# InSilicoModellingGroup/rdcFEs

Measured on AMD Instinct MI355X. Metric: elements_assembled_per_sec, higher is better.
Workload: dtype f64; 1 GPU; PIHNA TET4 K(119): 10110954 tets, 1728000 nodes, 5 unknowns, params run/PIHNA/input.dat (shipped), order=lex, state of SURVEY App. C (background (0,0,0,7170,0) of the shipped field file, tumour values inside a sphere r = 0.25; see state_sensitivity); scatter=rowgather, kernel_variant=auto, parallelism=single GPU, rank0_local_elements=10110954, rank0_nnz=639395950

## Files before the change

rdcfes_amd/csrc/rdc_capi.hip:

```cpp
#include <algorithm>
#include <cmath>
#include <cstdarg>
#include <cstdio>
#include <cstring>
#include <new>
#include <type_traits>
#include <utility>

#include "rdc_internal.h"
#include "rdc_const_rows.h"
#include "rdc_parts.h"
#include "rdc_tet4_ev.h"
#include "rdc_tet4_cl.h"
#include "rdc_solid.h"
#include "rdc_solve.h"

using namespace rdc;

namespace {

struct DevBuf { void* p = nullptr; size_t bytes = 0; bool owned = true; };

struct Buffers {
  struct { DevBuf conn, xyz, bptr, eslot, elem_order, first_mask, first_rhs, pair_elem, pair_local, node_pair_ptr, wg_node_ptr; } mesh;
// ... 58 lines not shown
  bool solid_part1_pending = false;
  int32_t n_materials = 0;
  int64_t n_sides = 0;
  int64_t field_count[RDC_FIELD_COUNT] = {};
};

thread_local char g_create_error[512] = "";

}

struct rdc_ctx {
  int device = 0;
  hipStream_t stream = nullptr;
  char err[512] = "";
  int strategy = RDC_SCATTER_AUTO;
  int variant = RDC_VARIANT_AUTO;
  int tet4_cl_mode = 0;
  int tet4_cl_active = 0;
  size_t tet4_cl_lds = 0;
  Options opt;
  MeshState ms;
  Buffers buf;
  ConstRows const_rows;
  hipEvent_t pack_event = nullptr;
  hipStream_t copy_stream = nullptr;
  hipEvent_t copy_fence = nullptr;
  static constexpr int N_TICKETS = 16;
  hipEvent_t ticket[N_TICKETS] = {};
  int next_ticket = 0;
  hipEvent_t solid_part1_event = nullptr;
  SolveScal* solve_rec = nullptr;
  int mg_omega_permille = MG_OMEGA_PERMILLE;
  int mg_smoother = 0;
  int mg_gs_fuse = 1;
  int ilu_factor_bits = 64;
  int solve_method = 0;
  int gmres_restart = GMRES_DEFAULT_RESTART;
  int gmres_refine = 0;
  GmresRec* gmres_rec = nullptr;
  bool timing = false;
  std::vector<hipEvent_t> ev;
  size_t ev_used = 0;
  size_t max_lds = 64 * 1024;
  int n_cu = 256;
};

// ... 409 lines not shown
  }
  a.val = (double*)c->buf.out.val.p;
  a.rhs = (double*)c->buf.out.rhs.p;
  a.stream = c->stream;
  a.colour_ptr = c->ms.prep.colour_ptr.data();
  a.n_colours = c->ms.prep.n_colours;
  a.n_wg = c->ms.prep.rowgather_ok ? (int)c->ms.prep.wg_node_ptr.size() - 1 : 0;
  a.lds_bytes = c->ms.prep.rg_lds_bytes;
  a.ev_start = nullptr;
  hipEvent_t ev_stop = nullptr;
  if (c->timing) {
    if ((rc = next_event_pair(c, &a.ev_start, &ev_stop))) return rc;
  }
  ConstRowsKey rows_key;
  bool capturing = false;
  if constexpr (std::is_same<M, Pihna>::value) {
    if (const_rows_path) {
      rows_key = const_rows_key(k);
      hipStreamCaptureStatus cs = hipStreamCaptureStatusNone;
      if (hipStreamIsCapturing(c->stream, &cs) != hipSuccess) { (void)hipGetLastError(); capturing = true; }
      else capturing = cs != hipStreamCaptureStatusNone;
      a.ev_rows = c->const_rows.rows(c->const_rows.mode, rows_key, plan.two_part == TwoPart::WHOLE ? 0 : part, c->opt.interior_nodes, capturing);
    }
  }
  hipError_t e = launch_specialised<M>(a, k);
  if (const_rows_path) c->const_rows.launched(a.ev_rows, rows_key, plan.two_part == TwoPart::WHOLE ? 0 : part, capturing, e == hipSuccess);
  if (e != hipSuccess) return fail(c, RDC_ERR_HIP, "kernel launch failed: %s", hipGetErrorString(e));
  if (c->timing) RDC_HIP(c, hipEventRecord(ev_stop, c->stream));
  return RDC_OK;
}

template <class F>
int with_part(rdc_ctx* c, int part, void* stream, F&& call) {
  if (!c) return RDC_ERR_INVALID;
  if (part < 0 || part > 2) return fail(c, RDC_ERR_INVALID, "part must be 0, 1 or 2");
  const int part0 = c->opt.part;
  const hipStream_t s0 = c->stream;
  c->opt.part = part;
  c->stream = (hipStream_t)stream;
  const int rc = call();
  c->opt.part = part0;
  c->stream = s0;
  return rc;
}
}

// ... 101 lines not shown
  if (!std::strcmp(key, "ilu_factor_bits")) {
    if (value != 64 && value != 32) return fail(c, RDC_ERR_INVALID, "ilu_factor_bits is 64 or 32, not %d", value);
    c->ilu_factor_bits = value;
    return RDC_OK;
  }
  if (!std::strcmp(key, "solve_method")) {
    if (value != 0 && value != 1) return fail(c, RDC_ERR_INVALID, "solve_method is 0 (BiCGStab) or 1 (GMRES), not %d", value);
    c->solve_method = value;
    return RDC_OK;
  }
  if (!std::strcmp(key, "gmres_restart")) {
    if (value < 1 || value > GMRES_MAX_RESTART) return fail(c, RDC_ERR_INVALID, "gmres_restart is 1 .. %d, not %d", GMRES_MAX_RESTART, value);
    c->gmres_restart = value;
    return RDC_OK;
  }
  if (!std::strcmp(key, "gmres_refine")) {
    if (value != 0 && value != 1) return fail(c, RDC_ERR_INVALID, "gmres_refine is 0 or 1, not %d", value);
    c->gmres_refine = value;
    return RDC_OK;
  }
  if (!std::strcmp(key, "const_rows")) {
    if (!const_rows_mode_ok(value)) return fail(c, RDC_ERR_INVALID, "%s", CONST_ROWS_REFUSED);
    c->const_rows.mode = value;
    return RDC_OK;
  }
  return options_set(c->opt, key, value, c->err, sizeof(c->err));
}

int rdc_get_scatter(const rdc_ctx* c, int* s) {
  if (!c || !s) return RDC_ERR_INVALID;
  int r = c->strategy;
  if (r == RDC_SCATTER_AUTO && c->ms.have_mesh) r = c->ms.prep.rowgather_ok ? RDC_SCATTER_ROWGATHER : RDC_SCATTER_COLOURED;
  *s = r;
  return RDC_OK;
}

int rdc_mesh_upload(rdc_ctx* c, int elem_type, int64_t n_elem, int64_t n_node, int64_t n_owned,
                    const uint32_t* conn, const double* xyz, int nvar) {
  if (!c) return RDC_ERR_INVALID;
  if (!conn || !xyz) return fail(c, RDC_ERR_INVALID, "null mesh arrays");
  int rc = set_device(c);
  if (rc) return rc;
  c->ms.have_mesh = false;
  c->const_rows.mesh_upload();
  const size_t budget = c->max_lds >= 64 * 1024 ? 50 * 1024 : c->max_lds / 2;
  std::string err = prep_build(elem_type, n_elem, n_node, n_owned, conn, nvar, budget, c->opt.block, c->ms.prep, c->opt.schedule != 0);
// ... 1415 lines not shown
```

rdcfes_amd/csrc/rdc_integrands.h:

```cpp
#ifndef RDC_INTEGRANDS_H
#define RDC_INTEGRANDS_H

#include <math.h>
#include "../../include/rdc_assembly.h"

#if defined(__HIPCC__)
#define RDC_HD __host__ __device__ __forceinline__
#else
#define RDC_HD inline
#endif

namespace rdc {

template <int NV, int NG>
struct Coef {
  double A[NV][NV];
  double B[NV][NV][NG];
  double D[NV][NV];
  double R[NV];
  double RG[NV][NG];
  RDC_HD void zero() {
    for (int a = 0; a < NV; a++) {
      R[a] = 0.0;
      for (int k = 0; k < NG; k++) RG[a][k] = 0.0;
// ... 36 lines not shown
  else if (EXP_MODE == 2) { pm1 = x; p = x * x; }
  else if (EXP_MODE == 3) { pm1 = x * x; p = pm1 * x; }
  else if (EXP_MODE == 4) { pm1 = x * x * x; p = pm1 * x; }
  else if (EXP_MODE == 25) { pm1 = x * sqrt(x); p = pm1 * x; }
  else {
    if (e == 3.0) { pm1 = x * x; p = pm1 * x; }
    else if (e == 2.0) { pm1 = x; p = x * x; }
    else if (e == 2.5) { pm1 = x * sqrt(x); p = pm1 * x; }
    else if (e == 4.0) { pm1 = x * x * x; p = pm1 * x; }
    else if (e == 1.0) { pm1 = 1.0; p = x; }
    else { p = rdc_pow_pos(x, e); pm1 = p * rcp(x); }
  }
}

struct PihnaK {
  double DT2, Lambda, Kappa, Ka, ek;
  double iKappa, mekK;
  double nec_c, nec_h, nec_v;
  double dif_c, tax_c, dif_h, tax_h, prod_c, c2h, h2c, h2n;
  double dif_v, tax_v, prod_v;
  double sec_c, sec_h, upt, dec;
  double Tn_c, Tn_h, Tn_v, Th2n, Tprod_c, Tc2h, Th2c, Tprod_v, Tdif_v, Tsec_c, Tsec_h, Tupt, Tdec;
  double Tdif_c, Ttax_c, Tdif_h, Ttax_h, Ttax_v;
};

struct Pihna {
  static constexpr int HEX_CL_POINTS = 1;
  static constexpr bool HEX_STAGED = false;
  static constexpr bool HEX_REF_GRADS = true;
  static constexpr int AUX_LOCAL_NODE = -1;
  static constexpr int NELEM = 0;
  RDC_HD static void grad_post(const PihnaK&, double (*)[3], const double*) {}
  static constexpr int NV = 5, NG = 4, NAUX = 0;
  static constexpr int FAST_EXP_MODE = 3;
  using K = PihnaK;
  using C = Coef<NV, NG>;
  RDC_HD static constexpr int grad_src(int k) { return k + 1; }
  RDC_HD static constexpr int row_order(int x) { return x; }
  RDC_HD static constexpr bool hasA(int a, int b) {
    return !((a == 0 && b == 4) || (a == 4 && b == 0) || (a == 1 && b == 4) || (a == 2 && b == 4));
  }
  RDC_HD static constexpr bool hasB(int a, int b, int k) {
    return b < 4 && ((a == 1 && (k == 0 || k == 2)) || (a == 2 && (k == 1 || k == 2)) || (a == 3 && (k == 2 || k == 3)));
  }
  RDC_HD static constexpr bool hasD(int a, int b) {
    return (a == 1 && (b == 1 || b == 3)) || (a == 2 && (b == 2 || b == 3)) || (a == 3 && (b == 3 || b == 4));
// ... 3 lines not shown
  }

  static inline K derive(const rdc_pihna_params& p) {
    K k;
    k.DT2 = p.time_step / 2.0;
    k.Lambda = p.cells_min_capacity;
    k.Kappa = p.cells_max_capacity;
    k.Ka = p.cytokines_max_capacity;
    k.ek = p.cells_max_capacity_exponent;
    k.iKappa = 1.0 / k.Kappa;
    k.mekK = -k.ek / k.Kappa;
    k.nec_c = p.necrosis_c / k.Kappa;
    k.nec_h = p.necrosis_h / k.Kappa;
    k.nec_v = p.necrosis_v / k.Kappa;
    k.dif_c = p.diffuse_c; k.tax_c = p.taxis_c; k.dif_h = p.diffuse_h; k.tax_h = p.taxis_h;
    k.prod_c = p.produce_c; k.c2h = p.switch_c2h; k.h2c = p.switch_h2c; k.h2n = p.switch_h2n;
    k.dif_v = p.diffuse_v; k.tax_v = p.taxis_v; k.prod_v = p.produce_v;
    k.sec_c = p.secrete_a_c; k.sec_h = p.secrete_a_h; k.upt = p.uptake_a_v; k.dec = p.decay_a;
    k.Tn_c = k.DT2 * k.nec_c; k.Tn_h = k.DT2 * k.nec_h; k.Tn_v = k.DT2 * k.nec_v; k.Th2n = k.DT2 * k.h2n;
    k.Tprod_c = k.DT2 * k.prod_c; k.Tc2h = k.DT2 * k.c2h; k.Th2c = k.DT2 * k.h2c; k.Tprod_v = k.DT2 * k.prod_v;
    k.Tdif_v = k.DT2 * k.dif_v; k.Tsec_c = k.DT2 * k.sec_c; k.Tsec_h = k.DT2 * k.sec_h; k.Tupt = k.DT2 * k.upt;
    k.Tdec = k.DT2 * k.dec;
    k.Tdif_c = k.DT2 * k.dif_c; k.Ttax_c = k.DT2 * k.tax_c; k.Tdif_h = k.DT2 * k.dif_h; k.Ttax_h = k.DT2 * k.tax_h; k.Ttax_v = k.DT2 * k.tax_v;
    return k;
  }
  static inline double exponent(const K& k) { return k.ek; }

  struct Pt {
    double n, c, h, v, a;
    double Tau, dT;
    double Ve, rV;
  };

  template <int EXP_MODE>
  RDC_HD static void point(const K& k, const double* u, const double* , Pt& s) {
    s.n = u[0]; s.c = u[1]; s.h = u[2]; s.v = u[3]; s.a = u[4];
    const double Te = (s.n + s.c + s.h + s.v) * k.iKappa;
    if (Te <= 0.0) { s.Tau = 1.0; s.dT = 0.0; }
    else if (Te >= 1.0) { s.Tau = 0.0; s.dT = 0.0; }
    else {
      double p, pm1;
      pow_pair<EXP_MODE>(1.0 - Te, k.ek, p, pm1);
      s.Tau = p;
      s.dT = k.mekK * pm1;
    }
    const double chv = s.c + s.h + s.v;
// ... 700 lines not shown
```

rdcfes_amd/csrc/rdc_internal.h:

```cpp
#ifndef RDC_INTERNAL_H
#define RDC_INTERNAL_H

#include <hip/hip_runtime.h>
#include <stdint.h>
#include <atomic>
#include <string>
#include <type_traits>
#include <vector>

#include "rdc_kernels.h"
#include "rdc_models.h"
#include "rdc_options.h"
#include "rdc_prep.h"

namespace rdc {

inline void dyn_lds_once(std::atomic<uint64_t>& done, const void* fn, int bytes) {
  int dev = 0;
  (void)hipGetDevice(&dev);
  const uint64_t bit = dev >= 0 && dev < 64 ? (1ull << dev) : 0;
  if (bit && (done.load(std::memory_order_relaxed) & bit)) return;
  (void)hipFuncSetAttribute(fn, hipFuncAttributeMaxDynamicSharedMemorySize, bytes);
  if (bit) done.fetch_or(bit, std::memory_order_relaxed);
}
// ... 42 lines not shown
};

struct LaunchArgs {
  MeshDev m;
  int nen, exp_mode;
  const double* u;
  const double* aux;
  const int64_t* hx_nl_ptr = nullptr;
  const uint32_t* hx_nlist = nullptr;
  const uint16_t* hx_ploc = nullptr;
  int hx_max_nodes = 0;
  const double* elem = nullptr;
  double* packed;
  int pack_part = 0;
  hipEvent_t pack_event = nullptr;
  Options opt;
  Plan plan;
  Rg2Dev rg2;
  EvDev ev;
  ClDev cl;
  int ev_grid = 0;
  int* ev_ticket = nullptr;
  int ev_rows = 5;
  long long* stamps = nullptr;
  double* val;
  double* rhs;
  hipStream_t stream;
  hipEvent_t ev_start;
  const int64_t* colour_ptr;
  int n_colours;
  int n_wg;
  size_t lds_bytes;
};

template <class M>
hipError_t launch_rd(const LaunchArgs& a, const typename M::K& k);
template <class M>
hipError_t launch_tet4_fast(const LaunchArgs& a, const typename M::K& k);
template <class M>
hipError_t launch_tet4_cl(const LaunchArgs& a, const typename M::K& k);
hipError_t pack_nodes_pihna(const LaunchArgs& a);
hipError_t launch_tet4_ev(const LaunchArgs& a, const PihnaK& k);
template <class M>
hipError_t launch_tet4_evc(const LaunchArgs& a, const typename M::K& k);

}
// ... 2 lines not shown
```

rdcfes_amd/csrc/rdc_tet4_ev.h:

```cpp
#ifndef RDC_TET4_EV_H
#define RDC_TET4_EV_H
#include "rdc_integrands.h"

namespace rdc {
namespace ev {

constexpr int NM = 16;
constexpr int NMG = 22;
constexpr int NBP = 256;
constexpr int MAXN = 16;
enum { M_E1, M_EoV, M_EPh, M_EQh, M_En, M_Ec, M_Eh, M_Ev, M_Ea, M_Ex, M_Ey, M_ETau, M_EdTc, M_Epv, M_Eg4, M_Edd,
       M_Xc, M_Yc, M_Zc, M_Xh, M_Yh, M_Zh };
constexpr bool symmetric_moment(int m) { return m != M_Epv; }
constexpr bool symmetric_moment_gen(int m) { return m != M_Epv && m != M_Edd && m != M_Xc && m != M_Yc && m != M_Xh && m != M_Yh; }

template <int EXP_MODE, class Sink, bool MIRROR = true, bool GEN = false>
RDC_HD void pihna_visit(const PihnaK& k, const double (&X)[4][3], const double (&U)[4][5], const int r, Sink& sink, const bool bg = false) {
  double e1[3], e2[3], e3[3];
#pragma unroll
  for (int d = 0; d < 3; d++) { e1[d] = X[1][d] - X[0][d]; e2[d] = X[2][d] - X[0][d]; e3[d] = X[3][d] - X[0][d]; }
  double g[4][3];
  g[1][0] = e2[1] * e3[2] - e2[2] * e3[1]; g[1][1] = e2[2] * e3[0] - e2[0] * e3[2]; g[1][2] = e2[0] * e3[1] - e2[1] * e3[0];
  g[2][0] = e3[1] * e1[2] - e3[2] * e1[1]; g[2][1] = e3[2] * e1[0] - e3[0] * e1[2]; g[2][2] = e3[0] * e1[1] - e3[1] * e1[0];
  g[3][0] = e1[1] * e2[2] - e1[2] * e2[1]; g[3][1] = e1[2] * e2[0] - e1[0] * e2[2]; g[3][2] = e1[0] * e2[1] - e1[1] * e2[0];
  const double det = e1[0] * g[1][0] + e1[1] * g[1][1] + e1[2] * g[1][2];
  const double inv = rcp(det), inv2 = inv * inv;
  const double adet = fabs(det);
#pragma unroll
  for (int d = 0; d < 3; d++) g[0][d] = -(g[1][d] + g[2][d] + g[3][d]);
  const double Wc = adet * (-2.0 / 15.0), Wh = adet * 0.075;
  const double a0 = Wc * (1.0 / 16.0), b36 = Wh * (1.0 / 36.0), w18 = Wh * (1.0 / 18.0);
  Pihna::Pt s[5];
  {
    double S[5];
#pragma unroll
    for (int v = 0; v < 5; v++) S[v] = (U[0][v] + U[1][v]) + (U[2][v] + U[3][v]);
#pragma unroll
    for (int q = 0; q < 5; q++) {
      double uq[5];
#pragma unroll
      for (int v = 0; v < 5; v++) uq[v] = (q == 0) ? 0.25 * S[v] : (S[v] * (1.0 / 6.0) + U[q == 0 ? 0 : q - 1][v] * (1.0 / 3.0));
      Pihna::point<EXP_MODE>(k, uq, nullptr, s[q]);
    }
  }
#define RDC_EV_SYM(m, beta)                                                                              \
  {                                                                                                      \
    const double Sm_ = a0 * beta[0] + b36 * ((beta[1] + beta[2]) + (beta[3] + beta[4]));                 \
    const double t_[4] = {w18 * beta[1], w18 * beta[2], w18 * beta[3], w18 * beta[4]};                   \
    _Pragma("unroll") for (int i = 0; i < 4; i++) if (i < r) {                                           \
      const double rb_ = Sm_ + t_[i];                                                                    \
      _Pragma("unroll") for (int j = 0; j < 4; j++) if (!MIRROR || j >= i) sink.mom(m, i, j, j == i ? rb_ + 3.0 * t_[i] : rb_ + t_[j]); \
    }                                                                                                    \
  }
#define RDC_EV_PT(name, expr) double name[5]; _Pragma("unroll") for (int q = 0; q < 5; q++) name[q] = (expr);
  const double o0 = Wc * 0.25, o6 = Wh * (1.0 / 6.0), o3 = Wh * (1.0 / 3.0);
#define RDC_EV_RHS(a, G)                                                             \
    {                                                                                \
      const double base_ = o0 * G[0] + o6 * ((G[1] + G[2]) + (G[3] + G[4]));         \
      _Pragma("unroll") for (int i = 0; i < 4; i++) if (i < r) sink.rhs(a, i, base_ + o3 * G[i + 1]); \
    }
  {
    double uav[5];
    {
      double g4[5];
#pragma unroll
      for (int q = 0; q < 5; q++) {
        const double raK = rcp(s[q].a + k.Ka);
        const double Ua = s[q].a * raK, Ua_da = raK - Ua * raK;
        uav[q] = Ua * s[q].v;
        g4[q] = -k.Tprod_v * (s[q].Tau * Ua_da * s[q].v);
      }
      RDC_EV_SYM(M_Eg4, g4)
    }
    {
      RDC_EV_PT(G3, s[q].v + k.Tprod_v * (s[q].Tau * uav[q]) - k.Tn_v * (s[q].v * s[q].n))
// ... 143 lines not shown
    }
  }
  if (!bg) {
    RDC_EV_PT(G, s[q].a + k.Tsec_c * s[q].c + k.Tsec_h * s[q].h - k.Tupt * (s[q].v * s[q].a) - k.Tdec * s[q].a)
    RDC_EV_RHS(4, G)
  }
#undef RDC_EV_RHS
  {
    const double one[5] = {1.0, 1.0, 1.0, 1.0, 1.0};
    RDC_EV_SYM(M_E1, one)
  }
  if (!bg) {
    { RDC_EV_PT(b, s[q].n) RDC_EV_SYM(M_En, b) }
    { RDC_EV_PT(b, s[q].c) RDC_EV_SYM(M_Ec, b) }
    { RDC_EV_PT(b, s[q].h) RDC_EV_SYM(M_Eh, b) }
    { RDC_EV_PT(b, s[q].dT * s[q].c) RDC_EV_SYM(M_EdTc, b) }
  }
  { RDC_EV_PT(b, s[q].v) RDC_EV_SYM(M_Ev, b) }
  if (k.Tupt != 0.0) { RDC_EV_PT(b, s[q].a) RDC_EV_SYM(M_Ea, b) }
  { RDC_EV_PT(b, s[q].Tau) RDC_EV_SYM(M_ETau, b) }
#undef RDC_EV_SYM
#undef RDC_EV_PT
}

RDC_HD bool pihna_background(const double (&U)[4][5]) {
  bool b = true;
#pragma unroll
  for (int j = 0; j < 4; j++) b = b && U[j][0] == 0.0 && U[j][1] == 0.0 && U[j][2] == 0.0 && U[j][4] == 0.0 && U[j][3] > 0.0;
  return b;
}

template <int NMT>
RDC_HD void pihna_expand(const PihnaK& k, const double (&e)[NMT], double (&o)[25]) {
  const double E1 = e[M_E1], EoV = e[M_EoV], EPh = e[M_EPh], EQh = e[M_EQh], En = e[M_En], Ec = e[M_Ec], Eh = e[M_Eh], Ev = e[M_Ev];
  const double x = e[M_Ex], y = e[M_Ey], pcj = k.Tprod_c * e[M_EdTc], pv = e[M_Epv];
  o[0] = E1 - k.Tn_c * Ec - k.Tn_h * Eh - k.Tn_v * Ev;
  o[1] = -(k.Tn_c * En + k.Th2n * EPh);
  o[2] = -(k.Tn_h * En + k.Th2n * EPh + k.Th2n * EoV);
  o[3] = k.Th2n * EQh - k.Tn_v * En;
  o[4] = 0.0;
  o[5] = k.Tn_c * Ec - pcj;
  o[6] = E1 - k.Tprod_c * e[M_ETau] - pcj + k.Tc2h * EoV + x + k.Tn_c * En;
  o[7] = x - pcj - k.Th2c * (E1 - EoV);
  o[8] = -(pcj + y);
  o[9] = 0.0;
  const double x2 = x - k.Th2n * EPh;
  o[10] = k.Tn_h * Eh;
  o[11] = -(k.Tc2h * EoV + x2);
  o[12] = E1 - x2 + k.Th2c * (E1 - EoV) + k.Tn_h * En + k.Th2n * EoV;
  o[13] = y - k.Th2n * EQh;
  o[14] = 0.0;
  o[15] = pv + k.Tn_v * Ev;
// ... 20 lines not shown
```

rdcfes_amd/csrc/rdc_tet4_ev.hip:

```cpp
#include "rdc_internal.h"
#include <type_traits>
#include "rdc_tet4_ev.h"
#include "rdc_ev_phases.h"

namespace rdc {

template <int ABL_>
struct EvSink {
  static constexpr int ABL = ABL_ == 4 ? 0 : ABL_;
  double* p[4][4];
  double* pr[4];
  double sum = 0.0;
  __device__ __forceinline__ void mom(int m, int i, int j, double v) {
    if (ABL == 0) __hip_atomic_fetch_add(p[i][j] + m * ev::NBP, v, __ATOMIC_RELAXED, __HIP_MEMORY_SCOPE_WORKGROUP);
    else if (ABL == 1) p[i][j][m * ev::NBP] = v;
    else sum += v;
  }
  __device__ __forceinline__ void rhs(int a, int i, double v) {
    if (ABL == 0) __hip_atomic_fetch_add(pr[i] + a * ev::MAXN, v, __ATOMIC_RELAXED, __HIP_MEMORY_SCOPE_WORKGROUP);
    else if (ABL == 1) pr[i][a * ev::MAXN] = v;
    else sum += v;
  }
};


namespace {
template <bool GEN, int NM>
__device__ __forceinline__ void ev_read_moments(const double* lds, const int blk, const int mirror, double (&e)[NM]) {
  constexpr auto sym = [](const int m) { return GEN ? ev::symmetric_moment_gen(m) : ev::symmetric_moment(m); };
  constexpr int NS = [=]() { int n = 0; for (int m = 0; m < NM; m++) n += sym(m); return n; }();
#pragma unroll
  for (int m = 0; m < NM; m++) e[m] = lds[m * ev::NBP + blk];
  if (mirror != blk) {
    double t[NS];
#pragma unroll
    for (int m = 0, x = 0; m < NM; m++)
      if (sym(m)) t[x++] = lds[m * ev::NBP + mirror];
    evl::lds_batch();
    evl::lds_land(t);
#pragma unroll
    for (int m = 0, x = 0; m < NM; m++)
      if (sym(m)) e[m] += t[x++];
  }
}
}

template <int EXP_MODE, int MINW, int ABL = 0, bool GEN = false, int NROW = 5>
__global__ void __launch_bounds__(256, MINW)
k_tet4_ev(const HostPrepEv::Desc* __restrict__ desc, const uint32_t* __restrict__ nlist, const uint32_t* __restrict__ vloc,
          const uint32_t* __restrict__ vslot, const HostPrepEv::Node* __restrict__ ntab, const uint8_t* __restrict__ bpart,
          const uint32_t* __restrict__ wg_perm, const PihnaK k, const double* __restrict__ rec, double* __restrict__ val,
          double* __restrict__ rhs, const int nls, const int wg_begin, const int xcd_n, const int stagger,
          long long* __restrict__ stamps, const int bg_skip) {
  static_assert(NROW == 4 || NROW == 5, "all five equation rows, or all but the a row");
  constexpr int BLOCK = 256, NP = 4;
  constexpr bool TL = ABL == 4;
  long long ts[11];
#define RDC_TS(x) if (TL) ts[x] = __builtin_amdgcn_s_memtime()
  RDC_TS(0);
  constexpr int NM = GEN ? ev::NMG : ev::NM, NBP = ev::NBP, MAXN = ev::MAXN;
  extern __shared__ __attribute__((aligned(16))) double lds[];
  __shared__ __attribute__((aligned(16))) HostPrepEv::Node snode[MAXN];
  typedef __attribute__((address_space(3))) void* lds_ptr;
  typedef const __attribute__((address_space(1))) void* glb_ptr;
  if (stagger > 0 && blockIdx.x < 1024u) {
    const unsigned lds_base = __builtin_amdgcn_s_getreg((7 << 11) | 6);
    const uint32_t slot = lds_base == 0 ? 0u : (lds_base < 144u ? 1u : 2u);
    for (uint32_t i = 0; i < slot * (uint32_t)stagger; i++) __builtin_amdgcn_s_sleep(16);
  }
  int wl = (int)blockIdx.x;
  if (xcd_n > 0) {
    const int q = xcd_n >> 3, rem = xcd_n & 7, x = wl & 7;
    wl = x * q + (x < rem ? x : rem) + (wl >> 3);
  }
  int w = wl + wg_begin;
  if (wg_perm) w = (int)wg_perm[w];
  const int tid = threadIdx.x, lane = tid & 63, wv = tid >> 6;
  double* const R = lds + NM * NBP;
  double* const recs = R + 5 * MAXN;
  evl::zero_slice<NM * NBP * 8>(lds, __builtin_amdgcn_readfirstlane(wv));
  if (tid < 5 * MAXN) lds[NM * NBP + tid] = 0.0;
  const int rounds = nls >> 6;
  uint32_t nid = 0;
  if (wv < rounds) nid = nlist[(size_t)w * nls + wv * 64 + lane];
  const uint32_t pl = vloc[(size_t)w * BLOCK + tid];
  const uint2 sl = reinterpret_cast<const uint2*>(vslot)[(size_t)w * BLOCK + tid];
  const HostPrepEv::Desc d = desc[w];
  const int mirror = (int)bpart[(size_t)w * NBP + tid];
  if (tid < MAXN) snode[tid] = ntab[(size_t)w * MAXN + tid];
  if (wv < rounds) {
    const char* src = reinterpret_cast<const char*>(rec) + (size_t)nid * (NP * 16);
#pragma unroll
    for (int p = 0; p < NP; p++)
      __builtin_amdgcn_global_load_lds((glb_ptr)(src + p * 16), (lds_ptr)evl::rec_at(recs, nls, p, wv * 64), 16, 0, 0);
  }
  RDC_TS(1);
  asm volatile("s_waitcnt vmcnt(0)" ::: "memory");
  RDC_TS(2);
  __syncthreads();
  RDC_TS(3);
  if (pl != evl::IDLE) {
    double X[4][3], U[4][5];
    int li[4];
#pragma unroll
    for (int j = 0; j < 4; j++) {
      li[j] = evl::vloc_pos(pl, j);
      double rr[2 * NP];
#pragma unroll
      for (int p = 0; p < NP; p++) {
        const double2 v2 = evl::rec_piece(recs, nls, p, li[j]);
        rr[2 * p] = v2.x; rr[2 * p + 1] = v2.y;
      }
      X[j][0] = rr[0]; X[j][1] = rr[1]; X[j][2] = rr[2];
#pragma unroll
      for (int v = 0; v < 5; v++) U[j][v] = rr[3 + v];
    }
    const int r = evl::vloc_rows(li, (int)d.nown);
    EvSink<ABL> sink;
    evl::aim(sink, lds, R, li, r, sl);
    const bool bg = bg_skip && __builtin_amdgcn_ballot_w64(!ev::pihna_background(U)) == 0;
    if (ABL != 3) ev::pihna_visit<EXP_MODE, EvSink<ABL>, true, GEN>(k, X, U, r, sink, bg);
    if (ABL == 2 && sink.sum == 1.2345e300) rhs[0] = sink.sum;
  }
  if (TL) asm volatile("s_waitcnt lgkmcnt(0)" ::: "memory");
  RDC_TS(4);
  __syncthreads();
  RDC_TS(5);
  double e[NM];
  const int bn = evl::block_node(tid), bs = evl::block_slot(tid);
  const bool has = bn < (int)d.nown && bs < (int)snode[bn < (int)d.nown ? bn : 0].len;
  if (has) ev_read_moments<GEN>(lds, tid, mirror, e);
  if (tid < (int)d.nown * 5) {
    const int n = tid / 5, a = tid - n * 5;
    rhs[(size_t)snode[n].node * 5 + a] = R[a * MAXN + n];
  }
  RDC_TS(6);
  __syncthreads();
  if (has) {
    double o[25];
    ev::pihna_expand(k, e, o);
    const int len = (int)snode[bn].len;
    double* dst = lds + snode[bn].obase + evl::seg_entry(5, len, 0, bs, 0);
#pragma unroll
    for (int a = 0; a < NROW; a++)
#pragma unroll
      for (int b = 0; b < 5; b++) dst[evl::seg_entry(5, len, a, 0, b)] = o[a * 5 + b];
  }
  RDC_TS(7);
  __syncthreads();
  RDC_TS(8);
  {
    const int wvu = __builtin_amdgcn_readfirstlane(wv);
    HostPrepEv::Node nd[4];
    evl::wave_nodes(snode, wvu, nd);
// ... 24 lines not shown
}
}
namespace {
struct EvqLists {
  static constexpr int PL = 0, SL = 1024, MISC = SL + 2048, MIRROR = MISC, SNODE = MISC + 256, DESC = MISC + 512, NL = MISC + 544;
  static constexpr int bytes(int nls) { return NL + 2 * nls * 4; }
};
}
template <int EXP_MODE, bool TL, bool GEN = false, int NROW = 5>
__global__ void __launch_bounds__(256, GEN ? 2 : 3)
k_tet4_evq(const HostPrepEv::Desc* __restrict__ desc, const uint32_t* __restrict__ nlist, const uint32_t* __restrict__ vloc,
           const uint32_t* __restrict__ vslot, const HostPrepEv::Node* __restrict__ ntab, const uint8_t* __restrict__ bpart,
           const PihnaK k, const double* __restrict__ rec, double* __restrict__ val, double* __restrict__ rhs, const int nls,
           const int wg_begin, const int wg_count, long long* __restrict__ stamps, const int bg_skip, int* __restrict__ ticket,
           const uint32_t* __restrict__ wg_perm) {
  static_assert(NROW == 4 || NROW == 5, "k_tet4_ev");
  constexpr int BLOCK = 256, NP = 4;
  constexpr int NM = GEN ? ev::NMG : ev::NM, NBP = ev::NBP, MAXN = ev::MAXN;
  extern __shared__ __attribute__((aligned(16))) double lds[];
  __shared__ __attribute__((aligned(16))) HostPrepEv::Node snode[MAXN];
  __shared__ uint8_t smirror[NBP];
  __shared__ int s_nown;
  __shared__ int s_tk[2];
  double* const R = lds + NM * NBP;
  double* const recs = R + 5 * MAXN;
  char* const lists = reinterpret_cast<char*>(recs + (size_t)NP * nls * 2);
  const int rounds = nls >> 6;
  auto lds_barrier = [&]() { asm volatile("s_waitcnt lgkmcnt(0)\n\ts_barrier" ::: "memory"); };
  const int wv = __builtin_amdgcn_readfirstlane((int)(threadIdx.x >> 6));
  constexpr int NONE = 0x7fffffff;
  int c0 = (int)blockIdx.x, c1 = c0 + (int)gridDim.x, c2 = c0 + 2 * (int)gridDim.x;
  auto cluster_of = [&](const int c) -> int { return c < wg_count ? (wg_perm ? (int)wg_perm[wg_begin + c] : wg_begin + c) : -1; };
  int w0c = cluster_of(c0), w1c = cluster_of(c1), w2c = cluster_of(c2);
#define RDC_TS(x) if (TL && stamps && c0 < wg_count && lane == 0) stamps[((int64_t)c0 * 4 + wv) * 12 + x] = __builtin_amdgcn_s_memtime()
  auto fetch = [&](const int w, const uint32_t nid, const int w2, const int nb2, const int lane) {
    if (wv < rounds) {
      const char* src = reinterpret_cast<const char*>(rec) + (size_t)nid * (NP * 16);
#pragma unroll
      for (int p = 0; p < NP; p++) evl_dma16(src + p * 16, evl::rec_at(recs, nls, p, wv * 64));
    }
    if (wv == 0) evl_dma16(reinterpret_cast<const char*>(vloc + (size_t)w * BLOCK) + lane * 16, lists + EvqLists::PL);
    else if (wv < 3) evl_dma16(reinterpret_cast<const char*>(vslot + (size_t)w * BLOCK * 2) + (wv - 1) * 1024 + lane * 16, lists + EvqLists::SL + (wv - 1) * 1024);
    else {
      if (lane < 34) {
        const char* src = lane < 16 ? reinterpret_cast<const char*>(bpart + (size_t)w * NBP) + lane * 16
                        : lane < 32 ? reinterpret_cast<const char*>(ntab + (size_t)w * MAXN) + (lane - 16) * 16
                                    : reinterpret_cast<const char*>(desc + w) + (lane - 32) * 16;
        evl_dma16(src, lists + EvqLists::MISC);
      }
      if (w2 >= 0 && lane < (nls >> 2)) evl_dma16(reinterpret_cast<const char*>(nlist + (size_t)w2 * nls) + lane * 16, lists + EvqLists::NL + nb2 * nls * 4);
    }
  };
  {
    uint32_t nid0 = 0;
    if (wv < rounds) nid0 = nlist[(size_t)w0c * nls + threadIdx.x];
    asm volatile("s_waitcnt vmcnt(0)" : "+v"(nid0)::"memory");
    fetch(w0c, nid0, w1c, 1, (int)(threadIdx.x & 63));
  }
  int tk = NONE;
  bool pending = false;
#pragma unroll 1
  for (int it = 0;; it++) {
    int lane;
    asm volatile("v_mbcnt_lo_u32_b32 %0, -1, 0\n\tv_mbcnt_hi_u32_b32 %0, -1, %0" : "=v"(lane));
    RDC_TS(0);
    evl::zero_slice<NM * NBP * 8>(lds, wv);
    if (wv * 64 + lane < 5 * MAXN) lds[NM * NBP + wv * 64 + lane] = 0.0;
    asm volatile("s_waitcnt vmcnt(0)" : "+v"(tk)::"memory");
    if (pending && wv == 0 && lane == 0) s_tk[0] = tk == NONE ? NONE : 3 * (int)gridDim.x + tk;
    RDC_TS(1);
    lds_barrier();
    RDC_TS(2);
    if (pending) { c2 = __builtin_amdgcn_readfirstlane(s_tk[0]); w2c = cluster_of(c2); }
    if (c0 >= wg_count) break;
    {
      const int tid = wv * 64 + lane;
      const uint32_t pl = *reinterpret_cast<const uint32_t*>(lists + EvqLists::PL + tid * 4);
      const uint2 sl = *reinterpret_cast<const uint2*>(lists + EvqLists::SL + tid * 8);
      const int nown = (int)reinterpret_cast<const HostPrepEv::Desc*>(lists + EvqLists::DESC)->nown;
      {
        const int blk = evl::block(((wv >> 1) << 3) | (lane & 7), ((wv & 1) << 3) | (lane >> 3));
        smirror[blk] = *reinterpret_cast<const uint8_t*>(lists + EvqLists::MIRROR + blk);
        if (tid < MAXN) snode[tid] = *reinterpret_cast<const HostPrepEv::Node*>(lists + EvqLists::SNODE + tid * 16);
        if (tid == 0) s_nown = nown;
      }
      if (pl != evl::IDLE) {
        double X[4][3], U[4][5];
        int li[4];
#pragma unroll
        for (int j = 0; j < 4; j++) {
          li[j] = evl::vloc_pos(pl, j);
          double rr[2 * NP];
#pragma unroll
          for (int p = 0; p < NP; p++) {
            const double2 v2 = evl::rec_piece(recs, nls, p, li[j]);
            rr[2 * p] = v2.x; rr[2 * p + 1] = v2.y;
          }
          X[j][0] = rr[0]; X[j][1] = rr[1]; X[j][2] = rr[2];
#pragma unroll
          for (int v = 0; v < 5; v++) U[j][v] = rr[3 + v];
        }
        const int r = evl::vloc_rows(li, nown);
        EvSink<0> sink;
        evl::aim(sink, lds, R, li, r, sl);
        const bool bg = bg_skip && __builtin_amdgcn_ballot_w64(!ev::pihna_background(U)) == 0;
        ev::pihna_visit<EXP_MODE, EvSink<0>, true, GEN>(k, X, U, r, sink, bg);
      }
    }
    RDC_TS(3);
    lds_barrier();
    RDC_TS(4);
    asm volatile("v_mbcnt_lo_u32_b32 %0, -1, 0\n\tv_mbcnt_hi_u32_b32 %0, -1, %0" : "=v"(lane));
    const int bn = ((wv >> 1) << 3) | (lane & 7), bs = ((wv & 1) << 3) | (lane >> 3), blk = evl::block(bn, bs);
    int nown = s_nown, mirror = (int)smirror[blk];
    uint32_t bn_len = reinterpret_cast<const uint32_t*>(snode + bn)[1], bn_obase = snode[bn].obase;
    uint32_t base8 = snode[8].obase;
    uint32_t nid = 0;
    if (c1 < wg_count && wv < rounds) nid = *reinterpret_cast<const uint32_t*>(lists + EvqLists::NL + (((it + 1) & 1) * nls + wv * 64 + lane) * 4);
    evl::lds_batch();
    evl::lds_land(nown, mirror); evl::lds_land(bn_len, bn_obase); evl::lds_land(base8, nid);
    nown = __builtin_amdgcn_readfirstlane(nown);
    base8 = __builtin_amdgcn_readfirstlane(base8);
    bn_len &= 0xFFFFu;
    if (c1 < wg_count) fetch(w1c, nid, w2c, it & 1, lane);
    tk = NONE;
    if (c2 < wg_count && wv == 0 && lane == 0) {
      const int one = 1;
      asm volatile("global_atomic_add %0, %1, %2, off sc0" : "=v"(tk) : "v"(ticket), "v"(one) : "memory");
    }
    pending = true;
    double e[NM];
    const bool has = bn < nown && bs < (int)bn_len;
#pragma unroll
    for (int m = 0; m < NM; m++) e[m] = 0.0;
    if (has) ev_read_moments<GEN>(lds, blk, mirror, e);
    {
      const int tid = wv * 64 + lane;
      if (tid < nown * 5) {
        const int n = tid / 5, a = tid - n * 5;
        rhs[(size_t)snode[n].node * 5 + a] = R[a * MAXN + n];
      }
    }
    double o[25];
    ev::pihna_expand(k, e, o);
    lds_barrier();
#pragma unroll 1
    for (int h = 0; h < 2; h++) {
      const int n0 = h * 8;
      if (n0 >= nown) break;
      const uint32_t base = h == 0 ? 0u : (base8 & ~1u);
      if ((wv >> 1) == h && has) {
        const int len = (int)bn_len;
        double* dst = lds + (bn_obase - base) + evl::seg_entry(5, len, 0, bs, 0);
#pragma unroll
        for (int a = 0; a < NROW; a++)
#pragma unroll
          for (int b = 0; b < 5; b++) dst[evl::seg_entry(5, len, a, 0, b)] = o[a * 5 + b];
      }
      evl::v4u_t raw[2];
      evl::wave_nodes_read(snode, n0 + wv, raw);
      HostPrepEv::Node ndh[2];
      evl::wave_nodes_land(raw, ndh);
      lds_barrier();
      const int n1 = nown < n0 + 8 ? nown : n0 + 8;
      const bool on[2] = {n0 + wv < n1, n0 + wv + 4 < n1};
      if (on[0]) evl::store_segments<25, 2, 5 * NROW>(lds, val, ndh, on, lane, base);
      lds_barrier();
    }
    RDC_TS(5);
    if (TL && lane == 0 && stamps) {
      long long* op = stamps + ((int64_t)c0 * 4 + wv) * 12;
      op[11] = (long long)__builtin_amdgcn_s_getreg((31 << 11) | 4) | ((long long)__builtin_amdgcn_s_getreg((31 << 11) | 20) << 32);
    }
    c0 = c1; c1 = c2; w0c = w1c; w1c = w2c;
  }
#undef RDC_TS
}


namespace {
template <int MODE, int MINW, int ABL, bool GEN>
hipError_t launch_ev(const LaunchArgs& a, const PihnaK& k, const int wg_count, const size_t lds_bytes) {
  const EvDev& E = a.ev;
  auto kern = k_tet4_ev<MODE, MINW, ABL, GEN, 5>;
  if constexpr (ABL == 0 || ABL == 4) {
    if (a.ev_rows == 4) kern = k_tet4_ev<MODE, MINW, ABL, GEN, 4>;
  } else if (a.ev_rows != 5) return hipErrorInvalidValue;
  hipLaunchKernelGGL(kern, dim3(wg_count), dim3(256), lds_bytes, a.stream, E.desc, E.nlist, E.vloc, E.vslot, E.ntab,
                     E.bpart, E.wg_perm, k, a.packed, a.val, a.rhs, E.nls, E.wg_begin, a.opt.xcd ? wg_count : 0, a.opt.stagger, a.stamps, a.opt.ev_background);
  return hipGetLastError();
}
template <int MODE, bool TL, bool GEN>
hipError_t launch_evq(const LaunchArgs& a, const PihnaK& k, const int wg_count, const int grid, const size_t lds_bytes) {
  const EvDev& E = a.ev;
  const auto kern = a.ev_rows == 4 ? k_tet4_evq<MODE, TL, GEN, 4> : k_tet4_evq<MODE, TL, GEN, 5>;
  hipLaunchKernelGGL(kern, dim3(grid), dim3(256), lds_bytes, a.stream, E.desc, E.nlist, E.vloc, E.vslot, E.ntab, E.bpart, k,
                     a.packed, a.val, a.rhs, E.nls, E.wg_begin, wg_count, a.stamps, a.opt.ev_background, a.ev_ticket + (a.pack_part == 2 ? 16 : 0), E.wg_perm);
  return hipGetLastError();
}
}

hipError_t launch_tet4_ev(const LaunchArgs& a, const PihnaK& k) {
  const EvDev& E = a.ev;
  hipError_t e = pack_nodes_pihna(a);
  if (e != hipSuccess) return e;
  if (a.ev_start) (void)hipEventRecord(a.ev_start, a.stream);
  const int wg_count = E.wg_count < 0 ? E.n_wg - E.wg_begin : E.wg_count;
  if (wg_count <= 0) return hipSuccess;
  const size_t acc = (size_t)(a.plan.ev_general ? ev::NMG : ev::NM) * ev::NBP + 5 * ev::MAXN + (size_t)4 * E.nls * 2;
  const bool cube = a.exp_mode == 3;
  const int evq_grid = a.opt.grid > 0 ? a.opt.grid : (a.ev_grid > 0 ? (a.plan.ev_general ? a.ev_grid : a.ev_grid / 2 * 3) : 768);
  if (a.opt.ev_resident && (!a.opt.ablate || (a.opt.ablate == 4 && !a.plan.ev_general)) && a.opt.ev_occupancy == 3 && !a.opt.xcd && a.opt.stagger == 0 &&
      (a.opt.grid > 0 || a.opt.ev_resident == 2 || (int64_t)wg_count >= 56 * (int64_t)evq_grid)) {
    const int grid = evq_grid > wg_count ? wg_count : evq_grid;
    const size_t bytes = acc * sizeof(double) + EvqLists::bytes(E.nls);
    if (!a.ev_ticket) return hipErrorInvalidValue;
    if (a.plan.ev_general) return cube ? launch_evq<3, false, true>(a, k, wg_count, grid, bytes) : launch_evq<0, false, true>(a, k, wg_count, grid, bytes);
    else if (a.opt.ablate == 4) return cube ? launch_evq<3, true, false>(a, k, wg_count, grid, bytes) : launch_evq<0, true, false>(a, k, wg_count, grid, bytes);
    else return cube ? launch_evq<3, false, false>(a, k, wg_count, grid, bytes) : launch_evq<0, false, false>(a, k, wg_count, grid, bytes);
  }
// ... 14 lines not shown
```

Measured before the change: 7.509 billion elements/s.

## Add wave-uniform background fast path folding constant-state moments per block

Adds a fast path in the TET4 element-visit assembly for waves whose elements all sit in the uniform background state, meaning zero cells and the same vasculature value at every node. Such waves skip the five per-quadrature-point material evaluations and emit only the geometric moment plus the diffusion and RHS terms. Background-dependent scalars are computed once, parked in shared memory, and folded into the moments at readout. This cuts transcendental and arithmetic work for the large background region, at the cost of an extra ballot and uniformity check per wave, added code size and register pressure, and a dependence on shared-memory state whose ordering is subtle.

```diff
diff --git a/rdcfes_amd/csrc/rdc_capi.hip b/rdcfes_amd/csrc/rdc_capi.hip
--- a/rdcfes_amd/csrc/rdc_capi.hip
+++ b/rdcfes_amd/csrc/rdc_capi.hip
@@ -104,6 +104,7 @@
   MeshState ms;
   Buffers buf;
   ConstRows const_rows;
+  int ev_uniform = 1;
   hipEvent_t pack_event = nullptr;
   hipStream_t copy_stream = nullptr;
   hipEvent_t copy_fence = nullptr;
@@ -559,6 +560,7 @@
       else capturing = cs != hipStreamCaptureStatusNone;
       a.ev_rows = c->const_rows.rows(c->const_rows.mode, rows_key, plan.two_part == TwoPart::WHOLE ? 0 : part, c->opt.interior_nodes, capturing);
     }
+    if (plan.path == Path::TET4_EV) a.ev_uniform = ev::pihna_uniform_allowed(k, plan.ev_general, c->opt.ev_background, c->opt.ablate, c->ev_uniform);
   }
   hipError_t e = launch_specialised<M>(a, k);
   if (const_rows_path) c->const_rows.launched(a.ev_rows, rows_key, plan.two_part == TwoPart::WHOLE ? 0 : part, capturing, e == hipSuccess);
@@ -706,6 +708,10 @@
   if (!std::strcmp(key, "const_rows")) {
     if (!const_rows_mode_ok(value)) return fail(c, RDC_ERR_INVALID, "%s", CONST_ROWS_REFUSED);
     c->const_rows.mode = value;
+    return RDC_OK;
+  }
+  if (!std::strcmp(key, "ev_uniform")) {
+    c->ev_uniform = value ? 1 : 0;
     return RDC_OK;
   }
   return options_set(c->opt, key, value, c->err, sizeof(c->err));
diff --git a/rdcfes_amd/csrc/rdc_integrands.h b/rdcfes_amd/csrc/rdc_integrands.h
--- a/rdcfes_amd/csrc/rdc_integrands.h
+++ b/rdcfes_amd/csrc/rdc_integrands.h
@@ -82,6 +82,7 @@
   double sec_c, sec_h, upt, dec;
   double Tn_c, Tn_h, Tn_v, Th2n, Tprod_c, Tc2h, Th2c, Tprod_v, Tdif_v, Tsec_c, Tsec_h, Tupt, Tdec;
   double Tdif_c, Ttax_c, Tdif_h, Ttax_h, Ttax_v;
+  double iKa;
 };
 
 struct Pihna {
@@ -131,6 +132,7 @@
     k.Tdif_v = k.DT2 * k.dif_v; k.Tsec_c = k.DT2 * k.sec_c; k.Tsec_h = k.DT2 * k.sec_h; k.Tupt = k.DT2 * k.upt;
     k.Tdec = k.DT2 * k.dec;
     k.Tdif_c = k.DT2 * k.dif_c; k.Ttax_c = k.DT2 * k.tax_c; k.Tdif_h = k.DT2 * k.dif_h; k.Ttax_h = k.DT2 * k.tax_h; k.Ttax_v = k.DT2 * k.tax_v;
+    k.iKa = 1.0 / k.Ka;
     return k;
   }
   static inline double exponent(const K& k) { return k.ek; }
diff --git a/rdcfes_amd/csrc/rdc_internal.h b/rdcfes_amd/csrc/rdc_internal.h
--- a/rdcfes_amd/csrc/rdc_internal.h
+++ b/rdcfes_amd/csrc/rdc_internal.h
@@ -88,6 +88,7 @@
   int ev_grid = 0;
   int* ev_ticket = nullptr;
   int ev_rows = 5;
+  bool ev_uniform = false;
   long long* stamps = nullptr;
   double* val;
   double* rhs;
diff --git a/rdcfes_amd/csrc/rdc_tet4_ev.h b/rdcfes_amd/csrc/rdc_tet4_ev.h
--- a/rdcfes_amd/csrc/rdc_tet4_ev.h
+++ b/rdcfes_amd/csrc/rdc_tet4_ev.h
@@ -15,7 +15,8 @@
 constexpr bool symmetric_moment_gen(int m) { return m != M_Epv && m != M_Edd && m != M_Xc && m != M_Yc && m != M_Xh && m != M_Yh; }
 
 template <int EXP_MODE, class Sink, bool MIRROR = true, bool GEN = false>
-RDC_HD void pihna_visit(const PihnaK& k, const double (&X)[4][3], const double (&U)[4][5], const int r, Sink& sink, const bool bg = false) {
+RDC_HD void pihna_visit_u(const PihnaK& k, const double (&X)[4][3], const double (&U)[4][5], const int r, Sink& sink, const bool bg, const bool uni,
+                          const double v0) {
   double e1[3], e2[3], e3[3];
 #pragma unroll
   for (int d = 0; d < 3; d++) { e1[d] = X[1][d] - X[0][d]; e2[d] = X[2][d] - X[0][d]; e3[d] = X[3][d] - X[0][d]; }
@@ -30,19 +31,6 @@
   for (int d = 0; d < 3; d++) g[0][d] = -(g[1][d] + g[2][d] + g[3][d]);
   const double Wc = adet * (-2.0 / 15.0), Wh = adet * 0.075;
   const double a0 = Wc * (1.0 / 16.0), b36 = Wh * (1.0 / 36.0), w18 = Wh * (1.0 / 18.0);
-  Pihna::Pt s[5];
-  {
-    double S[5];
-#pragma unroll
-    for (int v = 0; v < 5; v++) S[v] = (U[0][v] + U[1][v]) + (U[2][v] + U[3][v]);
-#pragma unroll
-    for (int q = 0; q < 5; q++) {
-      double uq[5];
-#pragma unroll
-      for (int v = 0; v < 5; v++) uq[v] = (q == 0) ? 0.25 * S[v] : (S[v] * (1.0 / 6.0) + U[q == 0 ? 0 : q - 1][v] * (1.0 / 3.0));
-      Pihna::point<EXP_MODE>(k, uq, nullptr, s[q]);
-    }
-  }
 #define RDC_EV_SYM(m, beta)                                                                              \
   {                                                                                                      \
     const double Sm_ = a0 * beta[0] + b36 * ((beta[1] + beta[2]) + (beta[3] + beta[4]));                 \
@@ -51,6 +39,39 @@
       const double rb_ = Sm_ + t_[i];                                                                    \
       _Pragma("unroll") for (int j = 0; j < 4; j++) if (!MIRROR || j >= i) sink.mom(m, i, j, j == i ? rb_ + 3.0 * t_[i] : rb_ + t_[j]); \
     }                                                                                                    \
+  }
+  if (!GEN && uni) {
+    const double u0[5] = {0.0, 0.0, 0.0, v0, 0.0};
+    Pihna::Pt s0;
+    Pihna::point<EXP_MODE>(k, u0, nullptr, s0);
+    {
+      const double one[5] = {1.0, 1.0, 1.0, 1.0, 1.0};
+      RDC_EV_SYM(M_Ea, one)
+    }
+    const double sdd = k.Tdif_v * (s0.v > k.Lambda ? s0.Tau : 0.0) * (Wc + 4.0 * Wh) * inv2;
+    const double fv = s0.v * (Wc * 0.25 + Wh);
+#pragma unroll
+    for (int i = 0; i < 4; i++) if (i < r) {
+      const double gs[3] = {sdd * g[i][0], sdd * g[i][1], sdd * g[i][2]};
+#pragma unroll
+      for (int j = 0; j < 4; j++)
+        if (!MIRROR || j >= i) sink.mom(M_Edd, i, j, gs[0] * g[j][0] + gs[1] * g[j][1] + gs[2] * g[j][2]);
+      sink.rhs(3, i, fv);
+    }
+    return;
+  }
+  Pihna::Pt s[5];
+  {
+    double S[5];
+#pragma unroll
+    for (int v = 0; v < 5; v++) S[v] = (U[0][v] + U[1][v]) + (U[2][v] + U[3][v]);
+#pragma unroll
+    for (int q = 0; q < 5; q++) {
+      double uq[5];
+#pragma unroll
+      for (int v = 0; v < 5; v++) uq[v] = (q == 0) ? 0.25 * S[v] : (S[v] * (1.0 / 6.0) + U[q == 0 ? 0 : q - 1][v] * (1.0 / 3.0));
+      Pihna::point<EXP_MODE>(k, uq, nullptr, s[q]);
+    }
   }
 #define RDC_EV_PT(name, expr) double name[5]; _Pragma("unroll") for (int q = 0; q < 5; q++) name[q] = (expr);
   const double o0 = Wc * 0.25, o6 = Wh * (1.0 / 6.0), o3 = Wh * (1.0 / 3.0);
@@ -240,12 +261,51 @@
 #undef RDC_EV_SYM
 #undef RDC_EV_PT
 }
+template <int EXP_MODE, class Sink, bool MIRROR = true, bool GEN = false>
+RDC_HD void pihna_visit(const PihnaK& k, const double (&X)[4][3], const double (&U)[4][5], const int r, Sink& sink, const bool bg = false,
+                        const double* uni = nullptr) {
+  pihna_visit_u<EXP_MODE, Sink, MIRROR, GEN>(k, X, U, r, sink, bg, uni != nullptr, uni != nullptr ? *uni : 0.0);
+}
 
 RDC_HD bool pihna_background(const double (&U)[4][5]) {
   bool b = true;
 #pragma unroll
   for (int j = 0; j < 4; j++) b = b && U[j][0] == 0.0 && U[j][1] == 0.0 && U[j][2] == 0.0 && U[j][4] == 0.0 && U[j][3] > 0.0;
   return b;
+}
+
+RDC_HD bool pihna_uniform(const double (&U)[4][5], const double v0) {
+  return U[0][3] == v0 && U[1][3] == v0 && U[2][3] == v0 && U[3][3] == v0;
+}
+
+inline bool pihna_uniform_allowed(const PihnaK& k, const bool gen, const int ev_background, const int ablate, const int ev_uniform) {
+  return !gen && k.Tupt == 0.0 && k.Ka > 0.0 && k.Ka <= 1.7976931348623157e308 && ev_background != 0 && (ablate == 0 || ablate == 4) &&
+         ev_uniform != 0;
+}
+
+template <int EXP_MODE>
+RDC_HD void pihna_uniform_scalars(const PihnaK& k, const double v0, double (&u)[3]) {
+  const double u0[5] = {0.0, 0.0, 0.0, v0, 0.0};
+  Pihna::Pt s0;
+  Pihna::point<EXP_MODE>(k, u0, nullptr, s0);
+  u[0] = s0.v;
+  u[1] = s0.Tau;
+  u[2] = -k.Tprod_v * (s0.Tau * k.iKa * s0.v);
+}
+
+template <int NMT>
+RDC_HD void pihna_fold_uniform(const double (&u)[3], double (&e)[NMT]) {
+  const double Eu = e[M_Ea];
+  e[M_E1] += Eu;
+  e[M_Ev] += u[0] * Eu;
+  e[M_ETau] += u[1] * Eu;
+  e[M_Eg4] += u[2] * Eu;
+}
+template <int EXP_MODE, int NMT>
+RDC_HD void pihna_fold_uniform(const PihnaK& k, const double v0, double (&e)[NMT]) {
+  double u[3];
+  pihna_uniform_scalars<EXP_MODE>(k, v0, u);
+  pihna_fold_uniform(u, e);
 }
 
 template <int NMT>
diff --git a/rdcfes_amd/csrc/rdc_tet4_ev.hip b/rdcfes_amd/csrc/rdc_tet4_ev.hip
--- a/rdcfes_amd/csrc/rdc_tet4_ev.hip
+++ b/rdcfes_amd/csrc/rdc_tet4_ev.hip
@@ -42,6 +42,53 @@
     for (int m = 0, x = 0; m < NM; m++)
       if (sym(m)) e[m] += t[x++];
   }
+}
+
+constexpr int EV_BG = 1, EV_UNI = 2;
+
+template <int EXP_MODE>
+__device__ __forceinline__ bool ev_wave_uniform(const PihnaK& k, const double (&U)[4][5], const double v0, double* park) {
+  if (!__builtin_isfinite(v0) || __builtin_amdgcn_ballot_w64(!ev::pihna_uniform(U, v0)) != 0) return false;
+  double u[3];
+  ev::pihna_uniform_scalars<EXP_MODE>(k, v0, u);
+  const uint64_t act = __builtin_amdgcn_ballot_w64(true);
+  if (__builtin_amdgcn_mbcnt_hi((uint32_t)(act >> 32), __builtin_amdgcn_mbcnt_lo((uint32_t)act, 0u)) == 0) {
+    park[0] = u[0]; park[1] = u[1]; park[2] = u[2];
+  }
+  return true;
+}
+
+template <int EXP_MODE, int ABL, bool GEN>
+__device__ __forceinline__ void ev_visit(const PihnaK& k, const uint32_t pl, const uint2 sl, const int nown, double* lds, double* R, const double* recs,
+                                         const int nls, const int bg_skip, double* park, EvSink<ABL>& sink) {
+  double X[4][3], U[4][5];
+  int li[4];
+#pragma unroll
+  for (int j = 0; j < 4; j++) {
+    li[j] = evl::vloc_pos(pl, j);
+    const double2 zn = evl::rec_piece(recs, nls, 1, li[j]), ch = evl::rec_piece(recs, nls, 2, li[j]), va = evl::rec_piece(recs, nls, 3, li[j]);
+    X[j][2] = zn.x;
+    U[j][0] = zn.y; U[j][1] = ch.x; U[j][2] = ch.y; U[j][3] = va.x; U[j][4] = va.y;
+  }
+  const int r = evl::vloc_rows(li, nown);
+  const bool bg = (bg_skip & EV_BG) && __builtin_amdgcn_ballot_w64(!ev::pihna_background(U)) == 0;
+  if (!GEN && bg && (bg_skip & EV_UNI)) {
+    const double v0 = evl::rec_piece(recs, nls, 3, 0).x;
+    if (ev_wave_uniform<EXP_MODE>(k, U, v0, park)) {
+      uint2 slu = sl;
+      int liu[4] = {li[0], li[1], li[2], li[3]};
+      asm volatile("" : "+v"(slu.x), "+v"(slu.y), "+v"(liu[0]), "+v"(liu[1]), "+v"(liu[2]), "+v"(liu[3]));
+#pragma unroll
+      for (int j = 0; j < 4; j++) { const double2 xy = evl::rec_piece(recs, nls, 0, liu[j]); X[j][0] = xy.x; X[j][1] = xy.y; }
+      evl::aim(sink, lds, R, liu, r, slu);
+      if (ABL != 3) ev::pihna_visit_u<EXP_MODE, EvSink<ABL>, true, GEN>(k, X, U, r, sink, true, true, v0);
+      return;
+    }
+  }
+#pragma unroll
+  for (int j = 0; j < 4; j++) { const double2 xy = evl::rec_piece(recs, nls, 0, li[j]); X[j][0] = xy.x; X[j][1] = xy.y; }
+  evl::aim(sink, lds, R, li, r, sl);
+  if (ABL != 3) ev::pihna_visit_u<EXP_MODE, EvSink<ABL>, true, GEN>(k, X, U, r, sink, bg, false, 0.0);
 }
 }
 
@@ -61,6 +108,7 @@
   constexpr int NM = GEN ? ev::NMG : ev::NM, NBP = ev::NBP, MAXN = ev::MAXN;
   extern __shared__ __attribute__((aligned(16))) double lds[];
   __shared__ __attribute__((aligned(16))) HostPrepEv::Node snode[MAXN];
+  __shared__ double s_uni[3];
   typedef __attribute__((address_space(3))) void* lds_ptr;
   typedef const __attribute__((address_space(1))) void* glb_ptr;
   if (stagger > 0 && blockIdx.x < 1024u) {
@@ -80,6 +128,7 @@
   double* const recs = R + 5 * MAXN;
   evl::zero_slice<NM * NBP * 8>(lds, __builtin_amdgcn_readfirstlane(wv));
   if (tid < 5 * MAXN) lds[NM * NBP + tid] = 0.0;
+  if (!GEN && (bg_skip & EV_UNI) && tid < 3) s_uni[tid] = 0.0;
   const int rounds = nls >> 6;
   uint32_t nid = 0;
   if (wv < rounds) nid = nlist[(size_t)w * nls + wv * 64 + lane];
@@ -100,26 +149,8 @@
   __syncthreads();
   RDC_TS(3);
   if (pl != evl::IDLE) {
-    double X[4][3], U[4][5];
-    int li[4];
-#pragma unroll
-    for (int j = 0; j < 4; j++) {
-      li[j] = evl::vloc_pos(pl, j);
-      double rr[2 * NP];
-#pragma unroll
-      for (int p = 0; p < NP; p++) {
-        const double2 v2 = evl::rec_piece(recs, nls, p, li[j]);
-        rr[2 * p] = v2.x; rr[2 * p + 1] = v2.y;
-      }
-      X[j][0] = rr[0]; X[j][1] = rr[1]; X[j][2] = rr[2];
-#pragma unroll
-      for (int v = 0; v < 5; v++) U[j][v] = rr[3 + v];
-    }
-    const int r = evl::vloc_rows(li, (int)d.nown);
     EvSink<ABL> sink;
-    evl::aim(sink, lds, R, li, r, sl);
-    const bool bg = bg_skip && __builtin_amdgcn_ballot_w64(!ev::pihna_background(U)) == 0;
-    if (ABL != 3) ev::pihna_visit<EXP_MODE, EvSink<ABL>, true, GEN>(k, X, U, r, sink, bg);
+    ev_visit<EXP_MODE, ABL, GEN>(k, pl, sl, (int)d.nown, lds, R, recs, nls, bg_skip, s_uni, sink);
     if (ABL == 2 && sink.sum == 1.2345e300) rhs[0] = sink.sum;
   }
   if (TL) asm volatile("s_waitcnt lgkmcnt(0)" ::: "memory");
@@ -130,6 +161,12 @@
   const int bn = evl::block_node(tid), bs = evl::block_slot(tid);
   const bool has = bn < (int)d.nown && bs < (int)snode[bn < (int)d.nown ? bn : 0].len;
   if (has) ev_read_moments<GEN>(lds, tid, mirror, e);
+  if constexpr (!GEN) {
+    if (has && (bg_skip & EV_UNI)) {
+      const double u[3] = {s_uni[0], s_uni[1], s_uni[2]};
+      ev::pihna_fold_uniform(u, e);
+    }
+  }
   if (tid < (int)d.nown * 5) {
     const int n = tid / 5, a = tid - n * 5;
     rhs[(size_t)snode[n].node * 5 + a] = R[a * MAXN + n];
@@ -200,6 +237,7 @@
   __shared__ uint8_t smirror[NBP];
   __shared__ int s_nown;
   __shared__ int s_tk[2];
+  __shared__ double s_uni[3];
   double* const R = lds + NM * NBP;
   double* const recs = R + 5 * MAXN;
   char* const lists = reinterpret_cast<char*>(recs + (size_t)NP * nls * 2);
@@ -229,6 +267,7 @@
       if (w2 >= 0 && lane < (nls >> 2)) evl_dma16(reinterpret_cast<const char*>(nlist + (size_t)w2 * nls) + lane * 16, lists + EvqLists::NL + nb2 * nls * 4);
     }
   };
+  if (!GEN && (bg_skip & EV_UNI) && threadIdx.x < 3) s_uni[threadIdx.x] = 0.0;
   {
     uint32_t nid0 = 0;
     if (wv < rounds) nid0 = nlist[(size_t)w0c * nls + threadIdx.x];
@@ -263,26 +302,8 @@
         if (tid == 0) s_nown = nown;
       }
       if (pl != evl::IDLE) {
-        double X[4][3], U[4][5];
-        int li[4];
-#pragma unroll
-        for (int j = 0; j < 4; j++) {
-          li[j] = evl::vloc_pos(pl, j);
-          double rr[2 * NP];
-#pragma unroll
-          for (int p = 0; p < NP; p++) {
-            const double2 v2 = evl::rec_piece(recs, nls, p, li[j]);
-            rr[2 * p] = v2.x; rr[2 * p + 1] = v2.y;
-          }
-          X[j][0] = rr[0]; X[j][1] = rr[1]; X[j][2] = rr[2];
-#pragma unroll
-          for (int v = 0; v < 5; v++) U[j][v] = rr[3 + v];
-        }
-        const int r = evl::vloc_rows(li, nown);
         EvSink<0> sink;
-        evl::aim(sink, lds, R, li, r, sl);
-        const bool bg = bg_skip && __builtin_amdgcn_ballot_w64(!ev::pihna_background(U)) == 0;
-        ev::pihna_visit<EXP_MODE, EvSink<0>, true, GEN>(k, X, U, r, sink, bg);
+        ev_visit<EXP_MODE, 0, GEN>(k, pl, sl, nown, lds, R, recs, nls, bg_skip, s_uni, sink);
       }
     }
     RDC_TS(3);
@@ -295,8 +316,11 @@
     uint32_t base8 = snode[8].obase;
     uint32_t nid = 0;
     if (c1 < wg_count && wv < rounds) nid = *reinterpret_cast<const uint32_t*>(lists + EvqLists::NL + (((it + 1) & 1) * nls + wv * 64 + lane) * 4);
+    double uf[3] = {0.0, 0.0, 0.0};
+    if (!GEN && (bg_skip & EV_UNI)) { uf[0] = s_uni[0]; uf[1] = s_uni[1]; uf[2] = s_uni[2]; }
     evl::lds_batch();
     evl::lds_land(nown, mirror); evl::lds_land(bn_len, bn_obase); evl::lds_land(base8, nid);
+    if (!GEN) evl::lds_land(uf);
     nown = __builtin_amdgcn_readfirstlane(nown);
     base8 = __builtin_amdgcn_readfirstlane(base8);
     bn_len &= 0xFFFFu;
@@ -312,6 +336,9 @@
 #pragma unroll
     for (int m = 0; m < NM; m++) e[m] = 0.0;
     if (has) ev_read_moments<GEN>(lds, blk, mirror, e);
+    if constexpr (!GEN) {
+      if (bg_skip & EV_UNI) ev::pihna_fold_uniform(uf, e);
+    }
     {
       const int tid = wv * 64 + lane;
       if (tid < nown * 5) {
@@ -357,6 +384,8 @@
 
 
 namespace {
+inline int ev_bg_skip(const LaunchArgs& a, const bool gen) { return a.opt.ev_background ? EV_BG | (a.ev_uniform && !gen ? EV_UNI : 0) : 0; }
+
 template <int MODE, int MINW, int ABL, bool GEN>
 hipError_t launch_ev(const LaunchArgs& a, const PihnaK& k, const int wg_count, const size_t lds_bytes) {
   const EvDev& E = a.ev;
@@ -365,7 +394,7 @@
     if (a.ev_rows == 4) kern = k_tet4_ev<MODE, MINW, ABL, GEN, 4>;
   } else if (a.ev_rows != 5) return hipErrorInvalidValue;
   hipLaunchKernelGGL(kern, dim3(wg_count), dim3(256), lds_bytes, a.stream, E.desc, E.nlist, E.vloc, E.vslot, E.ntab,
-                     E.bpart, E.wg_perm, k, a.packed, a.val, a.rhs, E.nls, E.wg_begin, a.opt.xcd ? wg_count : 0, a.opt.stagger, a.stamps, a.opt.ev_background);
+                     E.bpart, E.wg_perm, k, a.packed, a.val, a.rhs, E.nls, E.wg_begin, a.opt.xcd ? wg_count : 0, a.opt.stagger, a.stamps, ev_bg_skip(a, GEN));
   return hipGetLastError();
 }
 template <int MODE, bool TL, bool GEN>
@@ -373,7 +402,7 @@
   const EvDev& E = a.ev;
   const auto kern = a.ev_rows == 4 ? k_tet4_evq<MODE, TL, GEN, 4> : k_tet4_evq<MODE, TL, GEN, 5>;
   hipLaunchKernelGGL(kern, dim3(grid), dim3(256), lds_bytes, a.stream, E.desc, E.nlist, E.vloc, E.vslot, E.ntab, E.bpart, k,
-                     a.packed, a.val, a.rhs, E.nls, E.wg_begin, wg_count, a.stamps, a.opt.ev_background, a.ev_ticket + (a.pack_part == 2 ? 16 : 0), E.wg_perm);
+                     a.packed, a.val, a.rhs, E.nls, E.wg_begin, wg_count, a.stamps, ev_bg_skip(a, GEN), a.ev_ticket + (a.pack_part == 2 ? 16 : 0), E.wg_perm);
   return hipGetLastError();
 }
 }
```

New measurement: 7.617 billion elements/s, median of 6. 1.01x the previous value.
